# causalflow-ai/petit-kernel

Hardware: NVIDIA B200
Metric: FP4xBF16 GEMM algorithmic HBM GB/s, Llama-3.3-70B decoder-layer GEMM set (NVFP4, M=16) (higher is better)
Workload: dtype bf16

## Files before the change

petit-kernel_b200/csrc/capi.cu:

```cuda
#include "causalflow/petit/petit.h"
#include "fp4_gemm.h"
#include "layout.cuh"
#include "repack.h"

#include <atomic>
#include <cstdio>
#include <cstdlib>
#include <cstring>
#include <deque>
#include <map>
#include <mutex>
#include <set>
#include <tuple>
#include <utility>
#include <vector>

namespace {

using namespace petit;

constexpr uint64_t kFeatureGrid = 1;
constexpr uint64_t kElemNv = 1, kElemMx = 2;
constexpr uint64_t kMfmaF16 = 0, kMfmaBf16 = 1;
constexpr int kTokVariants[] = {16, 32, 64, 128, 256};
// ... 214 lines not shown
              cudaStream_t stream, const PetitFusedAllReduce *ar = nullptr,
              const PetitEpilogue *epi = nullptr, const gemm::GroupTable *table = nullptr) {
    if (ar) {
        if (m == 0 || n == 0 || k == 0 || m > gemm::kArMaxTokens) return PETIT_ERROR_PROBLEM_SHAPE;
        if (ar->world < 2 || ar->world > (int)gemm::kArMaxWorld || ar->rank < 0 ||
            ar->rank >= ar->world || !ar->state)
            return PETIT_ERROR_PROBLEM_SHAPE;
        for (int r = 0; r < ar->world; ++r)
            if (!ar->recv[r] || (reinterpret_cast<uintptr_t>(ar->recv[r]) & 15))
                return PETIT_ERROR_PROBLEM_SHAPE;
    }
    if (m == 0 || n == 0 || k == 0) return PETIT_OK;
    if (!hints) return PETIT_ERROR_KERNEL_SHAPE;
    const bool is_mx = force_mx || hints->b_type == PETIT_DTYPE_MXFP4_E2M1;

    Decoded d;
    if (solution_id == PETIT_SOLUTION_AUTO) {
        if (!problem_shape_ok(n, k)) return PETIT_ERROR_PROBLEM_SHAPE;
        if (hints->a_type != PETIT_DTYPE_FP16 && hints->a_type != PETIT_DTYPE_BF16)
            return PETIT_ERROR_PROBLEM_SHAPE;
        d = default_solution(is_mx, hints->a_type, m, n, k);
    } else {
        if (!decode_solution(solution_id, &d)) return PETIT_ERROR_KERNEL_SHAPE;
        if (force_mx) d.elem_b = kElemMx;
    }
    if (d.elem_b == kElemMx) {
        if (k % 32 != 0) return PETIT_ERROR_PROBLEM_SHAPE;
        if (hints->a_type != PETIT_DTYPE_BF16 || hints->c_type != PETIT_DTYPE_BF16 ||
            d.mfma != kMfmaBf16)
            return PETIT_ERROR_KERNEL_SHAPE;
    }
    if ((d.mfma == kMfmaBf16) != (hints->a_type == PETIT_DTYPE_BF16))
        return PETIT_ERROR_KERNEL_SHAPE;
    if (!problem_shape_ok(n, k)) return PETIT_ERROR_PROBLEM_SHAPE;

    if (((reinterpret_cast<uintptr_t>(a) | reinterpret_cast<uintptr_t>(c) |
          reinterpret_cast<uintptr_t>(b) | reinterpret_cast<uintptr_t>(scales)) & 15) != 0)
        return PETIT_ERROR_PROBLEM_SHAPE;

    Workspace ws;
    int num_sms = 0;
    int err = get_context(stream, &ws, &num_sms);
    if (err != PETIT_OK) return err;

    gemm::GemmArgs args;
    args.a = a;
    args.w = static_cast<const uint8_t *>(b);
    args.sc = static_cast<const uint8_t *>(scales);
    args.global_scale = global_scale_dev;
    args.c = c;
    args.ws_partials = ws.partials;
    args.ws_counters = ws.counters;
    args.ws_status = ws.counters + gemm::kMaxTiles;
    {
        static const unsigned long long wd = [] {
            const char *e = std::getenv("PETIT_WATCHDOG_MS");
            const long long ms = e ? std::atoll(e) : 2000;
            return (unsigned long long)(ms > 0 ? ms : 2000) * 1000000ull;
        }();
        args.watchdog_ns = wd;
    }
    args.m = m;
    args.n = n;
    args.k = k;
    args.trace = g_trace;
    args.bias = nullptr;
    args.residual = nullptr;
    args.act_silu_mul = 0;
    if (epi) {
        if (epi->activation != PETIT_ACT_NONE && epi->activation != PETIT_ACT_SILU_MUL)
            return PETIT_ERROR_KERNEL_SHAPE;
        if (epi->activation == PETIT_ACT_SILU_MUL) {
            if (n % layout::kTileN != 0 || epi->residual || ar) return PETIT_ERROR_PROBLEM_SHAPE;
            if (((n / 2) * 2) % 16 != 0) return PETIT_ERROR_PROBLEM_SHAPE;
        }
        if (((reinterpret_cast<uintptr_t>(epi->bias) | reinterpret_cast<uintptr_t>(epi->residual)) & 1) != 0)
            return PETIT_ERROR_PROBLEM_SHAPE;
        args.bias = epi->bias;
        args.residual = epi->residual;
        args.act_silu_mul = epi->activation == PETIT_ACT_SILU_MUL ? 1u : 0u;
    }
    args.ar_world = 0;
    args.ar_rank = 0;
    args.ar_two_shot = 0;
    args.ar_state = nullptr;
    for (auto &p : args.ar_recv) p = nullptr;
    if (ar) {
        args.ar_world = (uint32_t)ar->world;
        static const int two_shot_env = [] {
            const char *e = std::getenv("PETIT_AR_TWO_SHOT");
            return e ? std::atoi(e) : -1;
        }();
        const bool can_two_shot = ar->world == 4 || ar->world == 8 || ar->world == 2;
        args.ar_two_shot = !can_two_shot ? 0u
                           : two_shot_env >= 0 ? (uint32_t)(two_shot_env != 0)
                                               : (ar->world > 4 ? 1u : 0u);
        args.ar_rank = (uint32_t)ar->rank;
        args.ar_state = static_cast<unsigned *>(ar->state);
        for (int r = 0; r < ar->world; ++r) args.ar_recv[r] = static_cast<uint8_t *>(ar->recv[r]);
    }
    {
        static const int pdl = [] {
            const char *e = std::getenv("PETIT_PDL");
            return e ? std::atoi(e) : 1;
        }();
        args.use_pdl = (uint32_t)pdl;
// ... 457 lines not shown
```

petit-kernel_b200/csrc/fp4_gemm.cu:

```cuda
#include "fp4_gemm.h"
#include "dequant.cuh"
#include "layout.cuh"
#include "sm100_ptx.cuh"

#include <algorithm>
#include <atomic>
#include <cstdint>
#include <cstring>
#include <map>
#include <mutex>
#include <tuple>
#include <vector>
#include <cstddef>
#include <cstdlib>
#include <cuda_bf16.h>
#include <cuda_fp16.h>
#include <cuda_runtime.h>
#include <type_traits>

namespace petit::gemm {

using namespace petit::ptx;
using namespace petit::layout;
using namespace petit::dq;
// ... 153 lines not shown
    }
}
#ifdef PETIT_DEBUG_HOOKS
#define PETIT_DBG(flags, bit) ((flags) & (bit))
#else
#define PETIT_DBG(flags, bit) false
#endif
__device__ __forceinline__ void trace_stage(const GemmArgs &args, uint32_t stage, int ev) {
#ifndef PETIT_DEBUG_HOOKS
    (void)args; (void)stage; (void)ev;
    return;
#endif
    if (args.trace && blockIdx.x == 0 && stage < 64) {
        unsigned long long t;
        asm volatile("mov.u64 %0, %globaltimer;" : "=l"(t));
        args.trace[160 * 16 + stage * 8 + ev] = t;
    }
}
template <int N> __device__ __forceinline__ void setmaxnreg_inc() {
    asm volatile("setmaxnreg.inc.sync.aligned.u32 %0;" ::"n"(N));
}
template <int N> __device__ __forceinline__ void setmaxnreg_dec() {
    asm volatile("setmaxnreg.dec.sync.aligned.u32 %0;" ::"n"(N));
}
__device__ __forceinline__ void cluster_sync() {
    asm volatile("barrier.cluster.arrive.release.aligned;\n\tbarrier.cluster.wait.acquire.aligned;" ::
                     : "memory");
}
__device__ __forceinline__ void tma_load_3d_mc(void *smem_dst, const CUtensorMap *map, uint64_t *bar,
                                               int c0, int c1, int c2, uint16_t mask) {
    asm volatile("cp.async.bulk.tensor.3d.shared::cluster.global.tile.mbarrier::complete_tx::bytes"
                 ".multicast::cluster [%0], [%1, {%3, %4, %5}], [%2], %6;" ::"r"(smem_u32(smem_dst)),
                 "l"(map), "r"(smem_u32(bar)), "r"(c0), "r"(c1), "r"(c2), "h"(mask)
                 : "memory");
}
__device__ __forceinline__ void tc_commit_mc(uint64_t *bar, uint16_t mask) {
    asm volatile("tcgen05.commit.cta_group::1.mbarrier::arrive::one.shared::cluster.multicast::cluster"
                 ".b64 [%0], %1;" ::"r"(smem_u32(bar)),
                 "h"(mask)
                 : "memory");
}
__device__ __forceinline__ void griddep_wait() {
    asm volatile("griddepcontrol.wait;" ::: "memory");
}
__device__ __forceinline__ void griddep_launch_dependents() {
    asm volatile("griddepcontrol.launch_dependents;" ::: "memory");
}
__device__ __forceinline__ uint4 lds_v4(uint32_t addr) {
    uint4 v;
    asm volatile("ld.shared.v4.u32 {%0, %1, %2, %3}, [%4];"
                 : "=r"(v.x), "=r"(v.y), "=r"(v.z), "=r"(v.w)
                 : "r"(addr));
    return v;
}
__device__ __forceinline__ uint32_t lds_u32(uint32_t addr) {
    uint32_t v;
    asm volatile("ld.shared.u32 %0, [%1];" : "=r"(v) : "r"(addr));
    return v;
}
__device__ __forceinline__ float lds_f32(uint32_t addr) {
    float v;
    asm volatile("ld.shared.f32 %0, [%1];" : "=f"(v) : "r"(addr));
    return v;
}
__device__ __forceinline__ void sts_f32(uint32_t addr, float v) {
    asm volatile("st.shared.f32 [%0], %1;" ::"r"(addr), "f"(v) : "memory");
}
__device__ __forceinline__ uint32_t lds_u8(uint32_t addr) {
    uint32_t v;
    asm volatile("ld.shared.u8 %0, [%1];" : "=r"(v) : "r"(addr));
    return v;
}
__device__ __forceinline__ uint32_t lds_u16(uint32_t addr) {
    uint16_t v;
    asm volatile("ld.shared.u16 %0, [%1];" : "=h"(v) : "r"(addr));
    return v;
}
template <bool kBf16> __device__ __forceinline__ uint16_t to_bits16(float r) {
    if (kBf16) return __bfloat16_as_ushort(__float2bfloat16_rn(r));
    return __half_as_ushort(__float2half_rn(r));
}

__device__ __forceinline__ void mbar_wait_addr(uint32_t bar_addr, uint32_t parity) {
    asm volatile("{\n\t.reg .pred p;\n\t"
                 "W: mbarrier.try_wait.parity.shared::cta.b64 p, [%0], %1;\n\t"
                 "@p bra D;\n\tbra W;\n\tD:\n\t}" ::"r"(bar_addr),
                 "r"(parity)
                 : "memory");
}
__device__ __forceinline__ void mbar_arrive_addr(uint32_t bar_addr) {
    asm volatile("mbarrier.arrive.shared::cta.b64 _, [%0];" ::"r"(bar_addr) : "memory");
}

struct NoGroups {};
template <bool GR> struct GroupParam { using type = NoGroups; };
template <> struct GroupParam<true> { using type = GroupTable; };
__device__ __forceinline__ const GroupEntry &group_entry(const GroupTable &t, uint32_t i) { return t.e[i]; }
__device__ __forceinline__ GroupEntry group_entry(const NoGroups &, uint32_t) { return GroupEntry{}; }
__device__ __forceinline__ uint32_t group_tiles(const GroupTable &t) { return t.tiles; }
__device__ __forceinline__ uint32_t group_tiles(const NoGroups &) { return 0; }

static_assert(2 * sizeof(CUtensorMap) + sizeof(GemmArgs) + sizeof(GroupTable) <= 4096,
              "kernel parameters of the grouped GEMM exceed 4 KB: shrink kMaxGroupTiles");

template <int MODE, int NTOK, int KS, bool CL, bool AR = false, bool GR = false>
__global__ void __launch_bounds__(kNumThreads, 1)
// ... 119 lines not shown
                            asm volatile("mbarrier.complete_tx.relaxed.cta.shared::cta.b64 [%0], %1;" ::"r"(
                                             smem_u32(&bars->full[s])),
                                         "r"(sc_stage_bytes)
                                         : "memory");
                        else
                        bulk_g2s_hint(st + C::kActBytes + C::kWBytes, sc_src,
                                      sc_stage_bytes, &bars->full[s], pol_stream);
                    } else {
                        mbar_arrive_expect_tx(&bars->full_act[s], C::kActBytes);
                        if (PETIT_DBG(args.debug_flags, 4u))
                            asm volatile("mbarrier.complete_tx.relaxed.cta.shared::cta.b64 [%0], %1;" ::"r"(
                                             smem_u32(&bars->full_act[s])),
                                         "r"((uint32_t)C::kActBytes)
                                         : "memory");
                        else if (CL) {
#pragma unroll
                            for (int sl = 0; sl < C::kSubs; ++sl)
                                tma_load_3d_mc(st + sl * (NTOK * 128) +
                                                   cta_rank * (NTOK / 2) * 128,
                                               &tmap_act, &bars->full_act[s], 0,
                                               tok0 + cta_rank * (NTOK / 2),
                                               k_slab + sl, (uint16_t)3);
                        } else
                            tma_load_3d(st, &tmap_act, &bars->full_act[s], 0, tok0, k_slab);
                    }
                }
                __syncwarp();
                w_src += w_stage_bytes;
                sc_src += sc_stage_bytes;
                k_slab += C::kSubs;
            }
            u += g.kt1 - g.kt0;
        }
    } else if (warp == kMmaWarp || (C::kMmaWarps == 2 && warp == kMmaWarp2)) {
        constexpr uint32_t idesc = make_idesc_f16(
            C::kIsBf16 ? kFmtBF16 : kFmtF16, C::kIsBf16 ? kFmtBF16 : kFmtF16, 128, NTOK);
        constexpr int kHalfChains = C::kChains / C::kMmaWarps;
        const uint64_t bdesc0 = make_smem_desc_sw128(smem_u32(stage_base));
        auto mma_loop = [&](auto upper_tag) {
        constexpr bool kUpper = decltype(upper_tag)::value;
        uint64_t bdesc_s = bdesc0;
        uint32_t a_tmem = tmem_a0;
        uint32_t s = 0, ph = 0, ta = 0, ta_ph = 0, seg = 0;
        for (uint32_t u = u_begin; u < u_end; ++seg) {
            const Segment g = make_segment(sched, u, u_end);
            const uint32_t acc = seg % C::kNumAcc;
            const uint32_t acc_ph = (seg / C::kNumAcc) & 1;
            mbar_wait(&bars->acc_empty[acc], acc_ph ^ 1);
            tc_fence_after();
            const uint32_t d_tmem = tmem + acc * C::kAccBufCols;
            const uint32_t n_stage = (g.kt1 - g.kt0) * C::kStagesPerUnit;
            for (uint32_t i = 0; i < n_stage; ++i) {
                mbar_wait(&bars->full_act[s], ph);
#ifdef PETIT_DEBUG_HOOKS
                if (seg == 0 && i == 0 && lane == 0) trace_stamp(args, 3);
#endif
                mbar_wait(&bars->a_full[ta], ta_ph);
                tc_fence_after();
                if (elect_one()) {
#pragma unroll
                    for (int j = 0; j < KS / 16; ++j) {
                        if ((PETIT_KO & 1) && j >= 4) continue;
                        const int chain = j % C::kChains;
                        if (C::kMmaWarps == 2 && (chain >= kHalfChains) != kUpper) continue;
                        const uint64_t bdesc =
                            bdesc_s + (uint64_t)(((j / 4) * (NTOK * 128) + (j % 4) * 32) >> 4);
                        mma_f16_ts(d_tmem + chain * NTOK, a_tmem + j * 8, bdesc, idesc,
                                   (i != 0 || j >= C::kChains) ? 1u : 0u);
                    }
                    tc_commit(&bars->a_empty[ta]);
                    if (CL)
                        tc_commit_mc(&bars->empty_act[s], (uint16_t)3);
                    else
                        tc_commit(&bars->empty_act[s]);
                    if (i + 1 == n_stage) tc_commit(&bars->acc_full[acc]);
                }
                __syncwarp();
                bdesc_s += (uint64_t)(C::kStageBytes >> 4);
                a_tmem += C::kACols;
                if (++s == (uint32_t)C::kStages) { s = 0; ph ^= 1; bdesc_s = bdesc0; }
                if (++ta == (uint32_t)C::kAStages) { ta = 0; ta_ph ^= 1; a_tmem = tmem_a0; }
            }
            u += g.kt1 - g.kt0;
        }
        };
        if (C::kMmaWarps == 2 && warp == kMmaWarp2)
            mma_loop(std::true_type{});
        else
            mma_loop(std::false_type{});
        if (lane == 0 && warp == kMmaWarp) trace_stamp(args, 5);
    } else if (warp >= kFirstDequantWarp &&
               (warp - kFirstDequantWarp) / 4 < (uint32_t)C::kUsedSlices) {
        setmaxnreg_inc<kRegsDequant>();
        const uint32_t dw = warp - kFirstDequantWarp;
        const uint32_t quarter = warp % 4;
        const uint32_t kslice = dw / 4;
        const uint32_t row = quarter * 32 + lane;
        constexpr int kMyChunks = C::kChunks / C::kActiveSlices;
        constexpr int kScBytesPerChunk = C::kScPerSub / 2;
        const uint32_t group = kslice / C::kActiveSlices;
        const uint32_t c0 = (kslice % C::kActiveSlices) * kMyChunks;
        const uint32_t w_base = smem_u32(stage_base) + C::kActBytes;
        const uint32_t tmem_dst = tmem_a0 + ((quarter * 32) << 16) + c0 * 16;
        uint32_t s = 0, ph = 0, ta = 0, ta_ph = 1;
        uint32_t it_dbg = 0;
        if (args.skew_cycles) {
            const long long t0 = clock64();
            const long long wait = (long long)kslice * args.skew_cycles;
            while (clock64() - t0 < wait) {
            }
        }
        if (args.n % kTileN == 0) {
            constexpr uint32_t kG = C::kGroups;
            const uint32_t total = (u_end - u_begin) * C::kStagesPerUnit;
            const uint32_t bars_addr = smem_u32(bars);
            const uint32_t full_b = bars_addr + (uint32_t)offsetof(Barriers, full);
            const uint32_t aempty_b = bars_addr + (uint32_t)offsetof(Barriers, a_empty);
            constexpr uint32_t kFullToEmpty = (uint32_t)(offsetof(Barriers, empty) - offsetof(Barriers, full));
            constexpr int32_t kEmptyToFullA = (int32_t)offsetof(Barriers, a_full) - (int32_t)offsetof(Barriers, a_empty);
            const uint32_t lane_off = (c0 * kTileN + row) * 16;
            const uint32_t sc_lane_off = C::kWBytes + ((c0 / 2) * kTileN + row) * C::kScPerSub +
                                         (c0 & 1) * kScBytesPerChunk;
            const uint32_t st0 = w_base + lane_off, sc0 = w_base + sc_lane_off;
            const bool lane0 = lane == 0;
            auto stage_body = [&](uint32_t st_w, uint32_t st_sc, uint32_t fb, uint32_t ph2, uint32_t ab,
                                  uint32_t aph, uint32_t tm) {
                mbar_wait_addr(fb, ph2);
                uint4 q[kMyChunks];
#pragma unroll
                for (int ci = 0; ci < kMyChunks; ++ci) q[ci] = lds_v4(st_w + ci * (kTileN * 16));
                constexpr int kScLoads = kMyChunks >= 2 ? kMyChunks / 2 : 1;
                uint32_t scw[kScLoads];
#pragma unroll
                for (int p = 0; p < kScLoads; ++p) {
                    const uint32_t a = st_sc + p * (kTileN * C::kScPerSub);
                    if (kMyChunks >= 2)
                        scw[p] = C::kIsMx ? lds_u16(a) : lds_u32(a);
                    else
                        scw[p] = C::kIsMx ? lds_u8(a) : lds_u16(a);
                }
                mbar_wait_addr(ab, aph);
                tc_fence_after();
                bool any_two = false;
// ... 99 lines not shown
                    if (++s == C::kStages) { s = 0; ph ^= 1; }
                    if (++ta == C::kAStages) { ta = 0; ta_ph ^= 1; }
                    continue;
                }
                const uint32_t st = w_base + s * C::kStageBytes;
                mbar_wait(&bars->full[s], ph);
                if (threadIdx.x == kFirstDequantWarp * 32) trace_stage(args, it_dbg, 2);
                uint4 q[kMyChunks];
#pragma unroll
                for (int ci = 0; ci < kMyChunks; ++ci) q[ci] = lds_v4(st + w_off + ci * rows * 16);
                constexpr int kScLoads = kMyChunks >= 2 ? kMyChunks / 2 : 1;
                uint32_t scw[kScLoads];
#pragma unroll
                for (int p = 0; p < kScLoads; ++p) {
                    const uint32_t a = st + sc_off + p * rows * C::kScPerSub;
                    if (kMyChunks >= 2)
                        scw[p] = C::kIsMx ? lds_u16(a) : lds_u32(a);
                    else
                        scw[p] = C::kIsMx ? lds_u8(a) : lds_u16(a);
                }
                mbar_wait(&bars->a_empty[ta], ta_ph);
                tc_fence_after();
                if (threadIdx.x == kFirstDequantWarp * 32) trace_stage(args, it_dbg, 3);
#pragma unroll
                for (int ci = 0; ci < kMyChunks; ++ci) {
                    const uint32_t bits = scw[ci / 2] >> ((ci & 1) * 8 * kScBytesPerChunk);
                    bool two_step = false;
                    if (C::kIsMx) two_step = __any_sync(0xffffffffu, mx_needs_two_step(bits));
                    const uint32_t mult = chunk_multiplier<MODE>(bits, two_step);
                    uint32_t out[16];
                    if (PETIT_DBG(args.debug_flags, 2u)) {
#pragma unroll
                        for (int j = 0; j < 16; ++j) out[j] = q[ci].x + j;
                    } else
                    dequant_chunk<MODE>(q[ci], mult, two_step, out);
                    if (!PETIT_DBG(args.debug_flags, 16u))
                    tmem_st_x16(tmem_dst + ta * C::kACols + ci * 16, out);
                }
                tmem_wait_st();
                tc_fence_before();
                __syncwarp();
                if (threadIdx.x == kFirstDequantWarp * 32) trace_stage(args, it_dbg, 4);
                ++it_dbg;
                if (lane == 0) {
                    mbar_arrive(&bars->a_full[ta]);
                    mbar_arrive(&bars->empty[s]);
                }
                if (++s == C::kStages) { s = 0; ph ^= 1; }
                if (++ta == C::kAStages) { ta = 0; ta_ph ^= 1; }
            }
            u += g.kt1 - g.kt0;
        }
        if (threadIdx.x == kFirstDequantWarp * 32) trace_stamp(args, 4);
    } else if ((warp >= kFirstEpilogueWarp && warp < kFirstDequantWarp) ||
               (C::kEpiTeams > 1 && warp >= kFirstDequantWarp + 4 * C::kUsedSlices)) {
        setmaxnreg_inc<kRegsDequant>();
        const uint32_t quarter = warp % 4;
        const uint32_t team = warp < kFirstDequantWarp
                                  ? 0u
                                  : 1u + (warp - kFirstDequantWarp - 4 * C::kUsedSlices) / 4;
        const uint32_t ew_tid = (warp % 4) * 32 + lane;
        const bool lead = team == 0 && ew_tid == 0;
        constexpr int kAllEpiThreads = kNumEpilogueWarps * 32 * C::kEpiTeams;
        const int team_bar = kTeamBarId0 + (int)team;
        uint8_t *team_stage = out_stage + team * (C::kOutBufs * C::kOutStageBytes);
        bool ring_ready = false;
        const uint32_t row = quarter * 32 + lane;
        const uint32_t lane_base = (quarter * 32) << 16;
        griddep_wait();
        float gs = GR ? 0.f : *args.global_scale;
        gs *= epilogue_factor<MODE>();
        uint32_t ar_epoch = 0;
        if (AR)
            asm volatile("ld.relaxed.gpu.global.u32 %0, [%1];" : "=r"(ar_epoch) : "l"(args.ar_state) : "memory");
        const uint32_t sched_tiles_n = (args.n + kTileN - 1) / kTileN;
        uint32_t seg = 0;
        uint32_t out_buf = 0;
        for (uint32_t u = u_begin; u < u_end; ++seg) {
            const Segment g = make_segment(sched, u, u_end);
            const uint32_t rows = tile_rows(args.n, g.n_tile);
            const uint32_t acc = seg % C::kNumAcc;
            const uint32_t acc_ph = (seg / C::kNumAcc) & 1;
            const bool full_k = g.kt0 == 0 && g.kt1 == sched.k_tiles;
            uint32_t m0 = g.m_tile * NTOK;
            uint32_t m_valid = args.m - m0 < (uint32_t)NTOK ? args.m - m0 : NTOK;
            if (GR) {
                const GroupEntry &ge = group_entry(table, g.m_tile);
                m0 = ge.row0;
                m_valid = ge.rows;
                gs = __ldg(ge.gs) * epilogue_factor<MODE>();
            }

            const bool is_reducer = !full_k && g.kt0 == 0;
            const bool is_contrib = !full_k && g.kt0 != 0;
            float *slot = args.ws_partials + (size_t)blockIdx.x * (kTileN * NTOK);
            uint32_t b_first = sched_id, b_last = sched_id;
            if (is_reducer) b_last = sched.owner(g.tile * sched.k_tiles + sched.k_tiles - 1);
            const uint32_t out_tile = g.n_tile * sched.m_tiles + g.m_tile;

            const uint32_t pre_addr = pre_smem + row * 4;
            constexpr uint32_t kRingFit = (uint32_t)(C::kStages * C::kStageBytes) / (NTOK * kTileN * 4);
            const uint32_t ring_from = (is_reducer && b_last - b_first > 3u && b_last - b_first <= kRingFit) ? 0u : 16u;
            const bool last_seg = u + (g.kt1 - g.kt0) >= u_end;
            if (lead && last_seg) trace_stamp(args, 11);
            if (is_reducer) {
                if (lead) {
                    const uint32_t need = b_last - b_first;
                    uint32_t seen, spins = 0;
                    unsigned long long t_start = 0;
                    for (;;) {
                        asm volatile("ld.acquire.gpu.global.u32 %0, [%1];"
                                     : "=r"(seen)
                                     : "l"(args.ws_counters + out_tile)
                                     : "memory");
                        if (seen >= need) break;
                        if ((++spins & 0x3ff) == 0) {
                            unsigned long long now;
                            asm volatile("mov.u64 %0, %%globaltimer;" : "=l"(now));
                            if (t_start == 0) t_start = now;
                            if (now - t_start > args.watchdog_ns) {
                                atomicExch(args.ws_status, 1u + out_tile);
                                break;
                            }
                        }
                    }
                    if (last_seg) trace_stamp(args, 12);
                }
                named_bar_sync(kEpilogueBarId, kAllEpiThreads);
#pragma unroll 1
                for (uint32_t b = b_first + 1; b <= b_last && ring_from != 0 && team == 0; b += 2) {
                    const float *p = args.ws_partials +
                                     (size_t)(b * sched.n_mul + sched.n_add) * (kTileN * NTOK) + row;
                    const bool two = b + 1 <= b_last;
                    const float *p2 = p + (size_t)sched.n_mul * (kTileN * NTOK);
                    float x[16], y[16];
#pragma unroll
                    for (int j = 0; j < 16; ++j)
                        x[j] = (uint32_t)j < m_valid ? __ldcg(p + (size_t)j * kTileN) : 0.f;
#pragma unroll
                    for (int j = 0; j < 16; ++j)
                        y[j] = (two && (uint32_t)j < m_valid) ? __ldcg(p2 + (size_t)j * kTileN) : 0.f;
                    const bool first = b == b_first + 1;
#pragma unroll
                    for (int j = 0; j < 16; ++j) {
                        float acc = first ? 0.f : lds_f32(pre_addr + j * (kTileN * 4));
                        acc += x[j];
                        acc += y[j];
                        sts_f32(pre_addr + j * (kTileN * 4), acc);
                    }
                }
            }
            if (lead && last_seg) trace_stamp(args, 13);
            while (!mbar_try_wait(&bars->acc_full[acc], acc_ph)) __nanosleep(32);
            tc_fence_after();
            if (lead && last_seg) trace_stamp(args, 6);
            const uint32_t n_ring = (is_reducer && m_valid > ring_from)
                                        ? (b_last - b_first < kRingFit ? b_last - b_first : kRingFit)
                                        : 0u;
            if (n_ring && lead) {
                const uint32_t bytes = (m_valid - ring_from) * (kTileN * 4);
                mbar_arrive_expect_tx(&bars->part_full, n_ring * bytes);
                for (uint32_t i = 0; i < n_ring; ++i)
                    bulk_g2s(stage_base + (size_t)i * (NTOK * kTileN * 4) + ring_from * kTileN * 4,
                             args.ws_partials +
                                 (size_t)((b_first + 1 + i) * sched.n_mul + sched.n_add) *
                                     (kTileN * NTOK) +
                                 ring_from * kTileN,
                             bytes, &bars->part_full);
            }
            if (lead && seg == 1) trace_stamp(args, 9);
#pragma unroll 1
            for (int c0 = (int)team * 16; c0 < NTOK; c0 += 16 * C::kEpiTeams) {
                if ((uint32_t)c0 >= m_valid) break;
                float v[16];
                {
                    uint32_t r0[16];
                    tmem_ld_x16(tmem + lane_base + acc * C::kAccBufCols + c0, r0);
                    tmem_wait_ld();
#pragma unroll
                    for (int j = 0; j < 16; ++j) v[j] = __uint_as_float(r0[j]);
                }
                if (lead && last_seg && c0 == 0) trace_stamp(args, 14);
#pragma unroll
                for (int ch = 1; ch < C::kChains; ++ch) {
                    uint32_t r1[16];
                    tmem_ld_x16(tmem + lane_base + acc * C::kAccBufCols + ch * NTOK + c0, r1);
                    tmem_wait_ld();
#pragma unroll
                    for (int j = 0; j < 16; ++j) v[j] += __uint_as_float(r1[j]);
                }
                if (is_contrib) {
#pragma unroll
                    for (int j = 0; j < 16; ++j)
                        if ((uint32_t)(c0 + j) < m_valid)
                            __stcg(&slot[(size_t)(c0 + j) * kTileN + row], v[j]);
                    continue;
                }
                if (is_reducer && (uint32_t)c0 < ring_from) {
#pragma unroll
                    for (int j = 0; j < 16; ++j) v[j] += lds_f32(pre_addr + j * (kTileN * 4));
                } else if (is_reducer && !PETIT_DBG(args.debug_flags, 32u)) {
                    if (n_ring) {
                        if (!ring_ready) {
                            while (!mbar_try_wait(&bars->part_full, 0)) __nanosleep(32);
                            ring_ready = true;
                        }
#pragma unroll 1
                        for (uint32_t i = 0; i < n_ring; ++i) {
                            const uint32_t src = smem_u32(stage_base) + i * (NTOK * kTileN * 4) +
                                                 (uint32_t)c0 * (kTileN * 4) + row * 4;
                            uint32_t x[16];
#pragma unroll
                            for (int j = 0; j < 16; ++j) x[j] = lds_u32(src + j * (kTileN * 4));
#pragma unroll
                            for (int j = 0; j < 16; ++j) v[j] += __uint_as_float(x[j]);
                        }
                    }
#pragma unroll 1
                    for (uint32_t bb = b_first + 1 + n_ring; bb <= b_last; ++bb) {
                        const float *p = args.ws_partials +
                                         (size_t)(bb * sched.n_mul + sched.n_add) * (kTileN * NTOK) +
                                         (size_t)c0 * kTileN + row;
                        float x[16];
#pragma unroll
                        for (int j = 0; j < 16; ++j)
                            x[j] = (uint32_t)(c0 + j) < m_valid ? __ldcg(p + (size_t)j * kTileN) : 0.f;
#pragma unroll
                        for (int j = 0; j < 16; ++j) v[j] += x[j];
                    }
                }
#pragma unroll
                for (int j = 0; j < 16; ++j) v[j] *= gs;
                if (args.bias != nullptr || args.residual != nullptr) {
                    const uint32_t col = g.n_tile * kTileN + row;
                    if (row < rows) {
                        if (args.bias != nullptr) {
                            const uint16_t bb = static_cast<const uint16_t *>(args.bias)[col];
                            const float bv = C::kIsBf16 ? __uint_as_float((uint32_t)bb << 16)
                                                        : __half2float(__ushort_as_half(bb));
#pragma unroll
                            for (int j = 0; j < 16; ++j) v[j] += bv;
                        }
                        if (args.residual != nullptr) {
                            const uint16_t *rp = static_cast<const uint16_t *>(args.residual) +
                                                 (size_t)(m0 + c0) * args.n + col;
#pragma unroll
                            for (int j = 0; j < 16; ++j)
                                if ((uint32_t)(c0 + j) < m_valid) {
                                    const uint16_t rb = rp[(size_t)j * args.n];
                                    v[j] += C::kIsBf16 ? __uint_as_float((uint32_t)rb << 16)
                                                       : __half2float(__ushort_as_half(rb));
                                }
                        }
// ... 162 lines not shown
                            const uint16_t sb = to_bits16<C::kIsBf16>(gf / (1.0f + expf(-gf)));
                            const float sf = C::kIsBf16 ? __uint_as_float((uint32_t)sb << 16)
                                                        : __half2float(__ushort_as_half(sb));
                            r16[j] = to_bits16<C::kIsBf16>(sf * uf);
                        }
                    }
                    named_bar_sync(team_bar, kNumEpilogueWarps * 32);
                    if (row < 64) {
#pragma unroll
                        for (int j = 0; j < 16; ++j) stg[j * 64 + row] = r16[j];
                    }
                    fence_proxy_async();
                    named_bar_sync(team_bar, kNumEpilogueWarps * 32);
                    if (GR && m_valid - (uint32_t)c0 < 16u) {
                        const uint32_t j = ew_tid / 8, chunk = ew_tid % 8;
                        if ((uint32_t)c0 + j < m_valid)
                            *reinterpret_cast<uint4 *>(static_cast<uint16_t *>(args.c) +
                                                       (size_t)(m0 + c0 + j) * (args.n / 2) +
                                                       g.n_tile * 64 + chunk * 8) =
                                *reinterpret_cast<const uint4 *>(stg + j * 64 + chunk * 8);
                    } else if (ew_tid == 0) {
                        tma_store_2d(&tmap_out, stg, (int)(g.n_tile * 64), (int)(m0 + c0));
                        bulk_commit_group();
                    }
                    out_buf = out_buf == C::kOutBufs - 1 ? 0 : out_buf + 1;
                } else if (!PETIT_DBG(args.debug_flags, 64u)) {
                    uint16_t *stg = reinterpret_cast<uint16_t *>(team_stage + out_buf * C::kOutStageBytes);
#pragma unroll
                    for (int j = 0; j < 16; ++j) stg[j * kTileN + row] = to_bits16<C::kIsBf16>(v[j]);
                    if (!PETIT_DBG(args.debug_flags, 256u)) fence_proxy_async();
                    if (ew_tid == 0 && !PETIT_DBG(args.debug_flags, 128u))
                        bulk_wait_group_read<C::kOutBufs - 2>();
                    named_bar_sync(team_bar, kNumEpilogueWarps * 32);
                    if (GR && m_valid - (uint32_t)c0 < 16u) {
                        const uint32_t chunk = ew_tid % 16;
#pragma unroll
                        for (uint32_t j = ew_tid / 16; j < 16; j += 8)
                            if ((uint32_t)c0 + j < m_valid && chunk * 8 < rows)
                                *reinterpret_cast<uint4 *>(
                                    static_cast<uint16_t *>(args.c) + (size_t)(m0 + c0 + j) * args.n +
                                    g.n_tile * kTileN + chunk * 8) =
                                    *reinterpret_cast<const uint4 *>(stg + j * kTileN + chunk * 8);
                    } else if (ew_tid == 0 && !PETIT_DBG(args.debug_flags, 512u)) {
                        tma_store_2d(&tmap_out, stg, (int)(g.n_tile * kTileN), (int)(m0 + c0));
                        bulk_commit_group();
                    }
                    out_buf = out_buf == C::kOutBufs - 1 ? 0 : out_buf + 1;
                }
                if (lead && last_seg && c0 == 0) trace_stamp(args, 15);
            }
            tc_fence_before();
            __syncwarp();
            if (lane == 0) mbar_arrive(&bars->acc_empty[acc]);
            if (lead && seg == 1) trace_stamp(args, 10);

            if (is_contrib) {
                named_bar_sync(kEpilogueBarId, kAllEpiThreads);
                if (lead)
                    asm volatile("red.release.gpu.global.add.u32 [%0], 1;" ::"l"(
                                     args.ws_counters + out_tile)
                                 : "memory");
            } else if (is_reducer) {
                named_bar_sync(kEpilogueBarId, kAllEpiThreads);
                if (lead) args.ws_counters[out_tile] = 0;
            }
            u += g.kt1 - g.kt0;
        }
        if (ew_tid == 0) bulk_wait_group_read<0>();
    }

    if (threadIdx.x == kFirstEpilogueWarp * 32) trace_stamp(args, 7);
    tc_fence_before();
    if (CL)
        cluster_sync();
    else
        __syncthreads();
    if (threadIdx.x == 0) trace_stamp(args, 8);
    if (warp == kMmaWarp) tmem_dealloc(tmem, 512);
    if (AR && threadIdx.x == 0) {
        __threadfence();
        if (atomicAdd(args.ar_state + 1, 1u) == gridDim.x - 1) {
            args.ar_state[1] = 0;
            const uint32_t next = args.ar_state[0] + 1;
            args.ar_state[0] = next == kArCallPeriod ? 0u : next;
        }
    }
}

typedef CUresult (*EncodeTiledFn)(CUtensorMap *, CUtensorMapDataType, cuuint32_t, void *,
                                  const cuuint64_t *, const cuuint64_t *, const cuuint32_t *,
                                  const cuuint32_t *, CUtensorMapInterleave, CUtensorMapSwizzle,
                                  CUtensorMapL2promotion, CUtensorMapFloatOOBfill);

EncodeTiledFn get_encode_fn() {
    static EncodeTiledFn fn = []() -> EncodeTiledFn {
        void *p = nullptr;
        cudaDriverEntryPointQueryResult qres;
        if (cudaGetDriverEntryPoint("cuTensorMapEncodeTiled", &p, cudaEnableDefault, &qres) !=
                cudaSuccess ||
            qres != cudaDriverEntryPointSuccess)
            return nullptr;
        return reinterpret_cast<EncodeTiledFn>(p);
    }();
    return fn;
}

struct CutKey {
    uint32_t units, k_tiles, grid;
    int lat, late;
// ... 202 lines not shown
        e = cudaLaunchKernelEx(&cfg, kern, tmap, tmap_out, largs, *table);
    else
        e = cudaLaunchKernelEx(&cfg, kern, tmap, tmap_out, largs, NoGroups{});
    return e == cudaSuccess ? kLaunchOk : kLaunchCudaError;
}

template <int MODE> int launch_grouped_mode(const GemmArgs &args, int ntok, const GroupTable &table,
                                            int num_sms, cudaStream_t stream) {
    switch (ntok) {
    case 16: return launch_variant<MODE, 16, 256, false, false, true>(args, num_sms, stream, &table);
    case 32: return launch_variant<MODE, 32, 256, false, false, true>(args, num_sms, stream, &table);
    case 64: return launch_variant<MODE, 64, PETIT_KS_64, false, false, true>(args, num_sms, stream, &table);
    default: return kLaunchNoKernel;
    }
}

template <int MODE> int launch_mode(const GemmArgs &args, int ntok, int num_sms,
                                    cudaStream_t stream) {
    const uint32_t n_tiles = (args.n + kTileN - 1) / kTileN;
    const bool cluster_ok = args.use_cluster && n_tiles % 2 == 0 && args.n % kTileN == 0;
    if (args.ar_world > 1) {
        switch (ntok) {
        case 16: return launch_variant<MODE, 16, 256, false, true>(args, num_sms, stream);
        case 32: return launch_variant<MODE, 32, 256, false, true>(args, num_sms, stream);
        case 64: return launch_variant<MODE, 64, PETIT_KS_64, false, true>(args, num_sms, stream);
        default: return kLaunchNoKernel;
        }
    }
    switch (ntok) {
    case 16: return launch_variant<MODE, 16, 256>(args, num_sms, stream);
    case 32: return launch_variant<MODE, 32, 256>(args, num_sms, stream);
    case 64: return launch_variant<MODE, 64, PETIT_KS_64>(args, num_sms, stream);
    case 128:
        return cluster_ok ? launch_variant<MODE, 128, 128, true>(args, num_sms, stream)
                          : launch_variant<MODE, 128, 128>(args, num_sms, stream);
    case 256:
        return cluster_ok ? launch_variant<MODE, 256, 64, true>(args, num_sms, stream)
                          : launch_variant<MODE, 256, 64>(args, num_sms, stream);
    default: return kLaunchNoKernel;
    }
}

}

void debug_stream_k_cuts(uint32_t units, uint32_t k_tiles, uint32_t grid, int lat, int late,
                          int8_t *adj) {
    std::memset(adj, 0, kMaxGrid + 4);
    if (lat > 0 || late > 0) tilt_cuts(units, k_tiles, grid, lat, late, adj);
}

size_t workspace_partials_bytes() {
    return (size_t)kMaxGrid * kTileN * 256 * sizeof(float);
}
size_t workspace_counters_bytes() { return ((size_t)kMaxTiles + 1) * sizeof(unsigned); }

int launch_grouped(int mode, int ntok, const GemmArgs &args, const GroupTable &table, int num_sms,
                   cudaStream_t stream) {
    if (table.tiles == 0 || table.tiles > kMaxGroupTiles || args.ar_world > 1 || args.bias ||
        args.residual)
        return kLaunchBadShape;
    switch (mode) {
    case kModeNvF16: return launch_grouped_mode<kModeNvF16>(args, ntok, table, num_sms, stream);
    case kModeNvBf16: return launch_grouped_mode<kModeNvBf16>(args, ntok, table, num_sms, stream);
    case kModeMxBf16: return launch_grouped_mode<kModeMxBf16>(args, ntok, table, num_sms, stream);
    case kModeNvF16N: return launch_grouped_mode<kModeNvF16N>(args, ntok, table, num_sms, stream);
    default: return kLaunchNoKernel;
    }
}

int launch(int mode, int ntok, const GemmArgs &args, int num_sms, cudaStream_t stream) {
    switch (mode) {
    case kModeNvF16: return launch_mode<kModeNvF16>(args, ntok, num_sms, stream);
    case kModeNvBf16: return launch_mode<kModeNvBf16>(args, ntok, num_sms, stream);
    case kModeMxBf16: return launch_mode<kModeMxBf16>(args, ntok, num_sms, stream);
    case kModeNvF16N: return launch_mode<kModeNvF16N>(args, ntok, num_sms, stream);
    default: return kLaunchNoKernel;
    }
}

}
```

petit-kernel_b200/csrc/fp4_gemm.h:

```cpp
#pragma once

#include <cstddef>
#include <cstdint>
#include <cuda_runtime.h>

namespace petit::gemm {

enum : int { kModeNvF16 = 0, kModeNvBf16 = 1, kModeMxBf16 = 2, kModeNvF16N = 3 };
enum : int { kLaunchOk = 0, kLaunchBadShape = 1, kLaunchNoKernel = 2, kLaunchCudaError = 3 };

constexpr unsigned kMaxGrid = 160;
constexpr unsigned kMaxTiles = 1u << 20;

struct GemmArgs {
    const void *a;
    const uint8_t *w;
    const uint8_t *sc;
    const float *global_scale;
    void *c;
    const void *bias;
    const void *residual;
    uint32_t act_silu_mul;
    float *ws_partials;
    unsigned *ws_counters;
    unsigned *ws_status;
    unsigned long long watchdog_ns;
    uint32_t m, n, k;
    uint32_t debug_flags;
    uint32_t use_cluster;
    uint32_t use_pdl;
    uint32_t skew_cycles;
    unsigned long long *trace;
    int8_t cut_adj[kMaxGrid + 4];
    uint32_t ar_world, ar_rank;
    uint32_t ar_two_shot;
    uint8_t *ar_recv[8];
    unsigned *ar_state;
};

constexpr unsigned kArMaxWorld = 8;
constexpr unsigned kArMaxTokens = 64;
constexpr unsigned kArSlotBytes = 8192;
constexpr unsigned kArCallPeriod = 0xFFFFFFFEu;
inline size_t ar_recv_bytes(unsigned n) {
    return (size_t)2 * kArMaxWorld * ((n + 127) / 128) * (kArMaxTokens / 16) * kArSlotBytes;
}

struct GroupEntry {
    const uint8_t *w;
    const uint8_t *sc;
    const float *gs;
    uint32_t row0;
    uint32_t rows;
};
constexpr unsigned kMaxGroupTiles = 96;
struct GroupTable {
    uint32_t tiles;
    uint32_t pad;
    GroupEntry e[kMaxGroupTiles];
};

void debug_stream_k_cuts(uint32_t units, uint32_t k_tiles, uint32_t grid, int lat, int late,
                         int8_t *adj);

size_t workspace_partials_bytes();
size_t workspace_counters_bytes();

int launch(int mode, int ntok, const GemmArgs &args, int num_sms, cudaStream_t stream);
int launch_grouped(int mode, int ntok, const GemmArgs &args, const GroupTable &table, int num_sms,
                   cudaStream_t stream);

}
```

Baseline: 4678.

## Replace stream-K counter handshake with epoch-tagged partial packets for small NTOK

For NTOK<=64, contributor CTAs write their split-K partials as 16-byte packets that carry the call epoch next to each value, and reducers poll each packet directly. This removes the release-counter arrival, named barrier and spin on a tile counter before the reduction. A per-call epoch counter is added to the workspace and bumped by the last CTA to arrive. The cost is that partials take twice the bytes, the shared-memory ring holds half as many slots, and the reducer polls per packet. The epilogue also issues all TMEM chain loads before a single wait rather than one wait per chain.

```diff
diff --git a/petit-kernel_b200/csrc/capi.cu b/petit-kernel_b200/csrc/capi.cu
--- a/petit-kernel_b200/csrc/capi.cu
+++ b/petit-kernel_b200/csrc/capi.cu
@@ -290,6 +290,7 @@
     args.ws_partials = ws.partials;
     args.ws_counters = ws.counters;
     args.ws_status = ws.counters + gemm::kMaxTiles;
+    args.ws_epoch = ws.counters + gemm::kMaxTiles + 1;
     {
         static const unsigned long long wd = [] {
             const char *e = std::getenv("PETIT_WATCHDOG_MS");
diff --git a/petit-kernel_b200/csrc/fp4_gemm.cu b/petit-kernel_b200/csrc/fp4_gemm.cu
--- a/petit-kernel_b200/csrc/fp4_gemm.cu
+++ b/petit-kernel_b200/csrc/fp4_gemm.cu
@@ -229,6 +229,19 @@
                  : "=r"(v.x), "=r"(v.y), "=r"(v.z), "=r"(v.w)
                  : "r"(addr));
     return v;
+}
+__device__ __forceinline__ uint4 ld_relaxed_v4(const uint4 *p) {
+    uint4 v;
+    asm volatile("ld.relaxed.gpu.global.v4.u32 {%0, %1, %2, %3}, [%4];"
+                 : "=r"(v.x), "=r"(v.y), "=r"(v.z), "=r"(v.w)
+                 : "l"(p)
+                 : "memory");
+    return v;
+}
+__device__ __forceinline__ void st_relaxed_v4(uint4 *p, uint32_t a, uint32_t b, uint32_t c, uint32_t d) {
+    asm volatile("st.relaxed.gpu.global.v4.u32 [%0], {%1, %2, %3, %4};" ::"l"(p), "r"(a), "r"(b), "r"(c),
+                 "r"(d)
+                 : "memory");
 }
 __device__ __forceinline__ uint32_t lds_u32(uint32_t addr) {
     uint32_t v;
@@ -454,9 +467,6 @@
             const uint32_t n_stage = (g.kt1 - g.kt0) * C::kStagesPerUnit;
             for (uint32_t i = 0; i < n_stage; ++i) {
                 mbar_wait(&bars->full_act[s], ph);
-#ifdef PETIT_DEBUG_HOOKS
-                if (seg == 0 && i == 0 && lane == 0) trace_stamp(args, 3);
-#endif
                 mbar_wait(&bars->a_full[ta], ta_ph);
                 tc_fence_after();
                 if (elect_one()) {
@@ -485,12 +495,15 @@
             }
             u += g.kt1 - g.kt0;
         }
+        return seg;
         };
-        if (C::kMmaWarps == 2 && warp == kMmaWarp2)
-            mma_loop(std::true_type{});
-        else
-            mma_loop(std::false_type{});
-        if (lane == 0 && warp == kMmaWarp) trace_stamp(args, 5);
+        const uint32_t n_seg = (C::kMmaWarps == 2 && warp == kMmaWarp2) ? mma_loop(std::true_type{})
+                                                                        : mma_loop(std::false_type{});
+        if (lane == 0) trace_stamp(args, warp == kMmaWarp ? 5 : 9);
+        if (args.trace && warp == kMmaWarp && n_seg > 0) {
+            mbar_wait(&bars->acc_full[(n_seg - 1) % C::kNumAcc], ((n_seg - 1) / C::kNumAcc) & 1);
+            if (lane == 0) trace_stamp(args, 10);
+        }
     } else if (warp >= kFirstDequantWarp &&
                (warp - kFirstDequantWarp) / 4 < (uint32_t)C::kUsedSlices) {
         setmaxnreg_inc<kRegsDequant>();
@@ -696,9 +709,13 @@
             u += g.kt1 - g.kt0;
         }
         if (threadIdx.x == kFirstDequantWarp * 32) trace_stamp(args, 4);
+        if (C::kGroups > 1 && threadIdx.x == (kFirstDequantWarp + 4 * C::kActiveSlices) * 32)
+            trace_stamp(args, 3);
     } else if ((warp >= kFirstEpilogueWarp && warp < kFirstDequantWarp) ||
                (C::kEpiTeams > 1 && warp >= kFirstDequantWarp + 4 * C::kUsedSlices)) {
         setmaxnreg_inc<kRegsDequant>();
+        constexpr bool kPackets = NTOK <= 64;
+        static_assert(!kPackets || !CL, "packets: one CTA per scheduling unit");
         const uint32_t quarter = warp % 4;
         const uint32_t team = warp < kFirstDequantWarp
                                   ? 0u
@@ -717,6 +734,40 @@
         uint32_t ar_epoch = 0;
         if (AR)
             asm volatile("ld.relaxed.gpu.global.u32 %0, [%1];" : "=r"(ar_epoch) : "l"(args.ar_state) : "memory");
+        uint32_t pk_epoch = 0;
+        if (kPackets) {
+            asm volatile("ld.relaxed.gpu.global.u32 %0, [%1];" : "=r"(pk_epoch) : "l"(args.ws_epoch) : "memory");
+            named_bar_sync(kEpilogueBarId, kAllEpiThreads);
+            if (lead) {
+                uint32_t arrived;
+                asm volatile("atom.acq_rel.gpu.global.add.u32 %0, [%1], 1;"
+                             : "=r"(arrived) : "l"(args.ws_epoch + 1) : "memory");
+                if (arrived == gridDim.x - 1) {
+                    args.ws_epoch[1] = 0;
+                    args.ws_epoch[0] = pk_epoch + 1 == kArCallPeriod ? 0u : pk_epoch + 1;
+                }
+            }
+            pk_epoch += 1;
+        }
+        bool pk_gave_up = false;
+        auto pk_ok = [&](const uint4 &q) { return q.y == pk_epoch && q.w == pk_epoch; };
+        auto pk_poll = [&](const uint4 *src, uint4 q, uint32_t tile) {
+            uint32_t spins = 0;
+            unsigned long long t0 = 0;
+            while (!pk_ok(q) && !pk_gave_up) {
+                if ((++spins & 0xff) == 0) {
+                    unsigned long long now;
+                    asm volatile("mov.u64 %0, %%globaltimer;" : "=l"(now));
+                    if (t0 == 0) t0 = now;
+                    if (now - t0 > args.watchdog_ns) {
+                        atomicExch(args.ws_status, 1u + tile);
+                        pk_gave_up = true;
+                    }
+                }
+                q = ld_relaxed_v4(src);
+            }
+            return q;
+        };
         const uint32_t sched_tiles_n = (args.n + kTileN - 1) / kTileN;
         uint32_t seg = 0;
         uint32_t out_buf = 0;
@@ -738,6 +789,11 @@
             const bool is_reducer = !full_k && g.kt0 == 0;
             const bool is_contrib = !full_k && g.kt0 != 0;
             float *slot = args.ws_partials + (size_t)blockIdx.x * (kTileN * NTOK);
+            constexpr uint32_t kPkGroup = 8 * kTileN;
+            auto pk_src = [&](uint32_t b, int c0) {
+                return reinterpret_cast<const uint4 *>(args.ws_partials) +
+                       (size_t)b * (kTileN * NTOK / 2) + (uint32_t)c0 / 16 * kPkGroup + row;
+            };
             uint32_t b_first = sched_id, b_last = sched_id;
             if (is_reducer) b_last = sched.owner(g.tile * sched.k_tiles + sched.k_tiles - 1);
             const uint32_t out_tile = g.n_tile * sched.m_tiles + g.m_tile;
@@ -747,7 +803,35 @@
             const uint32_t ring_from = (is_reducer && b_last - b_first > 3u && b_last - b_first <= kRingFit) ? 0u : 16u;
             const bool last_seg = u + (g.kt1 - g.kt0) >= u_end;
             if (lead && last_seg) trace_stamp(args, 11);
-            if (is_reducer) {
+            if (is_reducer && kPackets) {
+#pragma unroll 1
+                for (uint32_t b = b_first + 1; b <= b_last && ring_from != 0; b += 2) {
+                    const bool two = b + 1 <= b_last;
+                    const uint4 *p = pk_src(b, 0), *p2 = pk_src(b + 1, 0);
+                    uint4 qx[8], qy[8];
+#pragma unroll
+                    for (int j = 0; j < 8; ++j) qx[j] = ld_relaxed_v4(p + j * kTileN);
+#pragma unroll
+                    for (int j = 0; j < 8; ++j) qy[j] = two ? ld_relaxed_v4(p2 + j * kTileN) : uint4{0, pk_epoch, 0, pk_epoch};
+                    const bool first = b == b_first + 1;
+#pragma unroll
+                    for (int j = 0; j < 8; ++j) {
+                        qx[j] = pk_poll(p + j * kTileN, qx[j], out_tile);
+                        qy[j] = pk_poll(p2 + j * kTileN, qy[j], out_tile);
+#pragma unroll
+                        for (int h = 0; h < 2; ++h) {
+                            const uint32_t t = 2 * j + h;
+                            const float x = t < m_valid ? __uint_as_float(h ? qx[j].z : qx[j].x) : 0.f;
+                            const float y = t < m_valid ? __uint_as_float(h ? qy[j].z : qy[j].x) : 0.f;
+                            float acc = first ? 0.f : lds_f32(pre_addr + t * (kTileN * 4));
+                            acc += x;
+                            acc += y;
+                            sts_f32(pre_addr + t * (kTileN * 4), acc);
+                        }
+                    }
+                }
+                if (lead && last_seg) trace_stamp(args, 12);
+            } else if (is_reducer) {
                 if (lead) {
                     const uint32_t need = b_last - b_first;
                     uint32_t seen, spins = 0;
@@ -798,10 +882,18 @@
             while (!mbar_try_wait(&bars->acc_full[acc], acc_ph)) __nanosleep(32);
             tc_fence_after();
             if (lead && last_seg) trace_stamp(args, 6);
+            constexpr uint32_t kRingSlots = kPackets ? kRingFit / 2 : kRingFit;
             const uint32_t n_ring = (is_reducer && m_valid > ring_from)
-                                        ? (b_last - b_first < kRingFit ? b_last - b_first : kRingFit)
+                                        ? (b_last - b_first < kRingSlots ? b_last - b_first : kRingSlots)
                                         : 0u;
             if (n_ring && lead) {
+                if (kPackets) {
+                    const uint32_t g0 = ring_from / 16, bytes = ((m_valid + 15) / 16 - g0) * kPkGroup * 16;
+                    mbar_arrive_expect_tx(&bars->part_full, n_ring * bytes);
+                    for (uint32_t i = 0; i < n_ring; ++i)
+                        bulk_g2s(stage_base + (size_t)i * (NTOK * kTileN * 8) + g0 * kPkGroup * 16,
+                                 pk_src(b_first + 1 + i, (int)ring_from) - row, bytes, &bars->part_full);
+                } else {
                 const uint32_t bytes = (m_valid - ring_from) * (kTileN * 4);
                 mbar_arrive_expect_tx(&bars->part_full, n_ring * bytes);
                 for (uint32_t i = 0; i < n_ring; ++i)
@@ -811,27 +903,37 @@
                                      (kTileN * NTOK) +
                                  ring_from * kTileN,
                              bytes, &bars->part_full);
+                }
             }
-            if (lead && seg == 1) trace_stamp(args, 9);
 #pragma unroll 1
             for (int c0 = (int)team * 16; c0 < NTOK; c0 += 16 * C::kEpiTeams) {
                 if ((uint32_t)c0 >= m_valid) break;
                 float v[16];
                 {
-                    uint32_t r0[16];
-                    tmem_ld_x16(tmem + lane_base + acc * C::kAccBufCols + c0, r0);
+                    uint32_t r[C::kChains][16];
+#pragma unroll
+                    for (int ch = 0; ch < C::kChains; ++ch)
+                        tmem_ld_x16(tmem + lane_base + acc * C::kAccBufCols + ch * NTOK + c0, r[ch]);
                     tmem_wait_ld();
 #pragma unroll
-                    for (int j = 0; j < 16; ++j) v[j] = __uint_as_float(r0[j]);
+                    for (int ch = 0; ch < C::kChains; ++ch)
+#pragma unroll
+                        for (int j = 0; j < 16; ++j) asm volatile("" : "+r"(r[ch][j]));
+#pragma unroll
+                    for (int j = 0; j < 16; ++j) v[j] = __uint_as_float(r[0][j]);
+#pragma unroll
+                    for (int ch = 1; ch < C::kChains; ++ch)
+#pragma unroll
+                        for (int j = 0; j < 16; ++j) v[j] += __uint_as_float(r[ch][j]);
                 }
                 if (lead && last_seg && c0 == 0) trace_stamp(args, 14);
-#pragma unroll
-                for (int ch = 1; ch < C::kChains; ++ch) {
-                    uint32_t r1[16];
-                    tmem_ld_x16(tmem + lane_base + acc * C::kAccBufCols + ch * NTOK + c0, r1);
-                    tmem_wait_ld();
-#pragma unroll
-                    for (int j = 0; j < 16; ++j) v[j] += __uint_as_float(r1[j]);
+                if (is_contrib && kPackets) {
+                    uint4 *dst = const_cast<uint4 *>(pk_src(blockIdx.x, c0));
+#pragma unroll
+                    for (int j = 0; j < 8; ++j)
+                        st_relaxed_v4(dst + j * kTileN, __float_as_uint(v[2 * j]), pk_epoch,
+                                      __float_as_uint(v[2 * j + 1]), pk_epoch);
+                    continue;
                 }
                 if (is_contrib) {
 #pragma unroll
@@ -843,6 +945,27 @@
                 if (is_reducer && (uint32_t)c0 < ring_from) {
 #pragma unroll
                     for (int j = 0; j < 16; ++j) v[j] += lds_f32(pre_addr + j * (kTileN * 4));
+                } else if (is_reducer && kPackets) {
+                    if (n_ring && !ring_ready) {
+                        while (!mbar_try_wait(&bars->part_full, 0)) __nanosleep(32);
+                        ring_ready = true;
+                    }
+#pragma unroll 1
+                    for (uint32_t i = 0; i < b_last - b_first; ++i) {
+                        const uint4 *src = pk_src(b_first + 1 + i, c0);
+                        uint4 q[8];
+#pragma unroll
+                        for (int j = 0; j < 8; ++j)
+                            q[j] = i < n_ring ? lds_v4(smem_u32(stage_base) + i * (NTOK * kTileN * 8) +
+                                                       ((uint32_t)c0 / 16 * kPkGroup + j * kTileN + row) * 16)
+                                              : ld_relaxed_v4(src + j * kTileN);
+#pragma unroll
+                        for (int j = 0; j < 8; ++j) {
+                            q[j] = pk_poll(src + j * kTileN, q[j], out_tile);
+                            v[2 * j] += __uint_as_float(q[j].x);
+                            v[2 * j + 1] += __uint_as_float(q[j].z);
+                        }
+                    }
                 } else if (is_reducer && !PETIT_DBG(args.debug_flags, 32u)) {
                     if (n_ring) {
                         if (!ring_ready) {
@@ -1111,9 +1234,9 @@
             tc_fence_before();
             __syncwarp();
             if (lane == 0) mbar_arrive(&bars->acc_empty[acc]);
-            if (lead && seg == 1) trace_stamp(args, 10);
-
-            if (is_contrib) {
+
+            if (kPackets) {
+            } else if (is_contrib) {
                 named_bar_sync(kEpilogueBarId, kAllEpiThreads);
                 if (lead)
                     asm volatile("red.release.gpu.global.add.u32 [%0], 1;" ::"l"(
@@ -1422,7 +1545,7 @@
 size_t workspace_partials_bytes() {
     return (size_t)kMaxGrid * kTileN * 256 * sizeof(float);
 }
-size_t workspace_counters_bytes() { return ((size_t)kMaxTiles + 1) * sizeof(unsigned); }
+size_t workspace_counters_bytes() { return ((size_t)kMaxTiles + 3) * sizeof(unsigned); }
 
 int launch_grouped(int mode, int ntok, const GemmArgs &args, const GroupTable &table, int num_sms,
                    cudaStream_t stream) {
diff --git a/petit-kernel_b200/csrc/fp4_gemm.h b/petit-kernel_b200/csrc/fp4_gemm.h
--- a/petit-kernel_b200/csrc/fp4_gemm.h
+++ b/petit-kernel_b200/csrc/fp4_gemm.h
@@ -24,6 +24,7 @@
     float *ws_partials;
     unsigned *ws_counters;
     unsigned *ws_status;
+    unsigned *ws_epoch;
     unsigned long long watchdog_ns;
     uint32_t m, n, k;
     uint32_t debug_flags;
```

Result: slower. 4289 (median of 6 runs) (-8.3%).
